# shaderko/velocity-asr

Measured on AMD Instinct MI355X. Metric: audio-sec/sec (RTFx) + frames/s, 5M model batch=32×10s @ 1/2/4/8 MI355X, higher is better.
Workload: dtype f32

## Files before the change

### velocity-asr_amd/csrc/gemm_rows.hip

```cpp
#include <type_traits>

#include "gemm_common.h"
#include "gemm_split.h"

namespace vasr {
namespace {

using namespace gemm;

typedef __attribute__((address_space(3))) void lds_void;

__device__ __forceinline__ void glds16(const void* src, void* dst_base) {
    const unsigned lds = (unsigned)(uintptr_t)(lds_void*)dst_base;
    unsigned keep;
    asm volatile("s_mov_b32 %0, m0\n\ts_mov_b32 m0, %1\n\ts_nop 0\n\tglobal_load_lds_dwordx4 %2, off\n\ts_mov_b32 m0, %0"
                 : "=&s"(keep) : "s"(lds), "v"(src) : "memory");
}

template <int N>
__device__ __forceinline__ void wait_vmcnt() {
    static_assert(N >= 0 && N < 64, "vmcnt range");
    __builtin_amdgcn_s_waitcnt((N & 15) | ((N >> 4) << 14) | (7 << 4) | (15 << 8));
}

#ifndef VASR_ROWS_ABLATE
#define VASR_ROWS_ABLATE 0
#endif
#ifndef VASR_ROWS_WAVES
#define VASR_ROWS_WAVES 8
#endif
#ifndef VASR_ROWS_DEPTH
#define VASR_ROWS_DEPTH 2
#endif
#ifndef VASR_ROWS_STORE_AUX
#define VASR_ROWS_STORE_AUX 2
#endif
constexpr int RW = VASR_ROWS_WAVES;
constexpr int DEPTH = VASR_ROWS_DEPTH;
constexpr int NSLOT = DEPTH + 1;
#ifndef VASR_ROWS_STORE_WAIT
#define VASR_ROWS_STORE_WAIT 1
#endif
#ifndef VASR_ROWS_MAX_GROUP
#define VASR_ROWS_MAX_GROUP 16
#endif
constexpr int MAX_GROUP = VASR_ROWS_MAX_GROUP;

__device__ __forceinline__ void wait_vmcnt_rt(int n) {
    switch (n) {
#define VASR_W(I) case I: wait_vmcnt<I>(); break;
#define VASR_W8(B) VASR_W(B) VASR_W(B + 1) VASR_W(B + 2) VASR_W(B + 3) VASR_W(B + 4) VASR_W(B + 5) VASR_W(B + 6) VASR_W(B + 7)
        VASR_W8(0) VASR_W8(8) VASR_W8(16) VASR_W8(24) VASR_W8(32) VASR_W8(40) VASR_W8(48) VASR_W8(56)
#undef VASR_W8
#undef VASR_W
        default: wait_vmcnt<0>();
    }
}

#ifdef VASR_ROWS_STAMPS
__device__ unsigned long long* g_rows_stamps;
#define VASR_STAMP(v) const unsigned long long v = __builtin_amdgcn_s_memtime()
#else
#define VASR_STAMP(v)
#endif

constexpr int NST = 16;
constexpr int OOB = 0x7FFFFFFC;

template <int EPI>
__device__ __forceinline__ void rows_epilogue(const GemmParams& p, __amdgpu_buffer_rsrc_t cbuf, int m0, int n0,
                                              const floatx16& acc, int r, int h, const float* __restrict__ bias_s,
                                              const float4* __restrict__ qp_s, int cfirst) {
    const int col = n0 + r;
    const bool col_ok = col < p.N;
    const int lc = col - cfirst;
    const float bv = p.bias ? bias_s[lc] : 0.0f;
    float4 qc = make_float4(0.f, 0.f, 0.f, 0.f);
    if (p.qp) qc = qp_s[lc];
    if constexpr (EPI == VASR_EPI_ARGMAX) {
        const int slot = n0 / 32;
#pragma unroll
        for (int i = 0; i < 16; ++i) {
            const int row = m0 + (i & 3) + 8 * (i >> 2) + 4 * h;
            float v = acc[i];
            if (p.bias) v = v + bv;
            if (p.qp) v = fake_quant(v, qc);
            const unsigned u = __float_as_uint(v);
            const unsigned ord = (u & 0x80000000u) ? ~u : (u | 0x80000000u);
            const unsigned long long k0 = col_ok ? ((unsigned long long)ord << 32) | (0xFFFFFFFFu - (unsigned)col) : 0ull;
            const unsigned long long key = gemm::max_u64_over_32_lanes(k0);
            const int off = (r == 31 && row < p.M) ? (row * (int)p.ldc + slot) * 8 : OOB;
            typedef unsigned u32x2 __attribute__((ext_vector_type(2)));
            const u32x2 kv = {(unsigned)key, (unsigned)(key >> 32)};
            if (!(VASR_ROWS_ABLATE & 2)) __builtin_amdgcn_raw_buffer_store_b64(kv, cbuf, off, 0, VASR_ROWS_STORE_AUX);
        }
        return;
    }
    auto body = [&](auto SPc) {
        constexpr int SP = decltype(SPc)::value;
        const bool sp = SP == 1 || (SP == 2 && col >= p.n_out);
#pragma unroll
        for (int i = 0; i < 16; ++i) {
            const int row = m0 + (i & 3) + 8 * (i >> 2) + 4 * h;
            const bool ok = col_ok && row < p.M;
            float v = acc[i];
            if (p.bias) v = v + bv;
            if (p.qp) v = fake_quant(v, qc);
            if constexpr (EPI == VASR_EPI_GELU) {
                v = gelu_fast(v);
            } else if constexpr (EPI == VASR_EPI_SOFTPLUS_FROM) {
                if constexpr (SP == 1) v = softplus20_fast(v);
                else if constexpr (SP == 2) v = sp ? softplus20_fast(v) : v;
            } else if constexpr (EPI == VASR_EPI_RESIDUAL) {
                v = v + p.aux[(int64_t)min(row, p.M - 1) * p.ld_aux + min(col, p.N - 1)];
            } else if constexpr (EPI == VASR_EPI_GELU_PE) {
                v = gelu_fast(v) + p.aux[(int64_t)min(row, p.M - 1) * p.ld_aux + min(col, p.N - 1)];
            }
            if (!(VASR_ROWS_ABLATE & 2))
                __builtin_amdgcn_raw_buffer_store_b32(__float_as_uint(v), cbuf, ok ? (row * (int)p.ldc + col) * 4 : OOB,
                                                      0, VASR_ROWS_STORE_AUX);
        }
    };
    if constexpr (EPI == VASR_EPI_SOFTPLUS_FROM) {
        if (n0 >= p.n_out) body(std::integral_constant<int, 1>());
        else if (n0 + 32 <= p.n_out) body(std::integral_constant<int, 0>());
        else body(std::integral_constant<int, 2>());
    } else {
        body(std::integral_constant<int, 0>());
    }
}

template <int KS, int EPI>
__global__ __launch_bounds__(64 * RW, 1) void gemm_rows_kernel(GemmParams p, int n_groups, int chunks_per_group) {
    constexpr int CHUNK = KS * 3 * 1024;
    constexpr int DW = 4;
    constexpr int NDMA = 3 * KS / DW;
    static_assert((3 * KS) % DW == 0 && RW % DW == 0, "whole DMA pieces per loader wave");
    __shared__ __attribute__((aligned(16))) char wb0[CHUNK];
    __shared__ __attribute__((aligned(16))) char wb1[CHUNK];
    __shared__ __attribute__((aligned(16))) char wb2[CHUNK];
    __shared__ __attribute__((aligned(16))) char wb3[NSLOT > 3 ? CHUNK : 16];
    __shared__ float bias_s[MAX_GROUP * 32];
    __shared__ float4 qp_s[MAX_GROUP * 32];

    const int nblk = (int)gridDim.x;
    const int id = blockIdx.x;
    const int q8 = nblk / 8, r8 = nblk % 8, xg = id % 8;
    const int w = (xg < r8 ? xg * (q8 + 1) : r8 * (q8 + 1) + (xg - r8) * q8) + id / 8;
    const int rb = w / n_groups, ng = w - rb * n_groups;
    const int NT = (p.N + 31) / 32;
    const int c0 = ng * chunks_per_group;
    const int nc = min(chunks_per_group, NT - c0);
    if (nc <= 0) return;

    const int tid = threadIdx.x;
    const int lane = tid & 63;
    const int wave = tid >> 6;
    const int r = lane & 31, h = lane >> 5;
    const int wave_u = __builtin_amdgcn_readfirstlane(wave);
    const int m0 = rb * 32 * RW + wave * 32;
    const int cfirst = c0 * 32;

    const float* __restrict__ arow = p.A + (int64_t)min(m0 + r, p.M - 1) * p.lda;
    float4 xa[KS][2];
#pragma unroll
    for (int ks = 0; ks < KS; ++ks)
#pragma unroll
        for (int u = 0; u < 2; ++u) {
            const int k = 16 * ks + 8 * h + 4 * u;
            const float4 v = *reinterpret_cast<const float4*>(arow + min(k, p.K - 4));
            xa[ks][u] = k < p.K ? v : make_float4(0.f, 0.f, 0.f, 0.f);
        }
    for (int i = tid; i < nc * 32; i += 64 * RW) {
        const int col = min(cfirst + i, p.N - 1);
        if (p.bias) bias_s[i] = p.bias[col];
        if (p.qp) qp_s[i] = p.qp[col];
    }
    bf16x8 a[KS][3];
#pragma unroll
    for (int ks = 0; ks < KS; ++ks) split8(xa[ks][0], xa[ks][1], a[ks][0], a[ks][1], a[ks][2]);

    const char* __restrict__ Wx = reinterpret_cast<const char*>(p.Wx);
    auto slot = [&](int i) -> char* { return i == 0 ? wb0 : i == 1 ? wb1 : i == 2 ? wb2 : wb3; };
    const bool loader = wave_u < DW;
    auto issue = [&](int j) {
        if (!loader) return;
        const char* src = Wx + (int64_t)(c0 + j) * CHUNK + lane * 16;
        char* dst = slot(j % NSLOT);
#pragma unroll
        for (int i = 0; i < NDMA; ++i) {
            const int piece = i * DW + wave_u;
            glds16(src + piece * 1024, dst + piece * 1024);
        }
    };
    for (int j = 0; j < DEPTH && j < nc; ++j) issue(j);

    const int c_bytes = (EPI == VASR_EPI_ARGMAX ? 8 : 4) * ((p.M - 1) * (int)p.ldc + (EPI == VASR_EPI_ARGMAX ? NT : p.N));
    const __amdgpu_buffer_rsrc_t cbuf = __builtin_amdgcn_make_buffer_rsrc(p.C, 0, c_bytes, 0x00020000);
    floatx16 acc[2];
#ifdef VASR_ROWS_STAMPS
    unsigned long long st_wait = 0, st_bar = 0, st_epi = 0, st_dma = 0, st_mfma = 0;
    VASR_STAMP(st_begin);
#endif
    auto step = [&](auto Sc, int j) {
        constexpr int S = decltype(Sc)::value;
        int n_vm = 0;
        if (!loader && !(VASR_ROWS_ABLATE & 2)) n_vm = VASR_ROWS_STORE_WAIT ? NST * max(0, j - max(j - DEPTH + 1, 1)) : 63;
        VASR_STAMP(t0);
        wait_vmcnt_rt(min(n_vm, 63));
        VASR_STAMP(t1);
        if (!(VASR_ROWS_ABLATE & 8)) __builtin_amdgcn_s_barrier();
        VASR_STAMP(t2);
        const char* wb = slot((VASR_ROWS_ABLATE & 4) ? min(j, DEPTH - 1) : j % NSLOT) + lane * 16;
        bf16x8 wf[2][3];
#pragma unroll
        for (int pl = 0; pl < 3; ++pl) wf[0][pl] = *reinterpret_cast<const bf16x8*>(wb + pl * 1024);
        if (j >= 1) rows_epilogue<EPI>(p, cbuf, m0, (c0 + j - 1) * 32, acc[S ^ 1], r, h, bias_s, qp_s, cfirst);
        VASR_STAMP(t3);
        if (j + DEPTH < nc && !(VASR_ROWS_ABLATE & 4)) issue(j + DEPTH);
        VASR_STAMP(t4);
        floatx16 c;
#pragma unroll
        for (int i = 0; i < 16; ++i) c[i] = 0.f;
#pragma unroll
        for (int ks = 0; ks < KS; ++ks) {
            const int cur = ks & 1;
            if (ks + 1 < KS) {
#pragma unroll
                for (int pl = 0; pl < 3; ++pl)
                    wf[cur ^ 1][pl] = *reinterpret_cast<const bf16x8*>(wb + ((ks + 1) * 3 + pl) * 1024);
            }
            __builtin_amdgcn_sched_barrier(0);
            if constexpr (VASR_ROWS_ABLATE & 1) {
                c[0] += (float)a[ks][0][0] * (float)wf[cur][0][0] + (float)a[ks][2][1] * (float)wf[cur][2][1];
                continue;
            }
            c = __builtin_amdgcn_mfma_f32_32x32x16_bf16(a[ks][2], wf[cur][0], c, 0, 0, 0);
            c = __builtin_amdgcn_mfma_f32_32x32x16_bf16(a[ks][0], wf[cur][2], c, 0, 0, 0);
            c = __builtin_amdgcn_mfma_f32_32x32x16_bf16(a[ks][1], wf[cur][1], c, 0, 0, 0);
            c = __builtin_amdgcn_mfma_f32_32x32x16_bf16(a[ks][1], wf[cur][0], c, 0, 0, 0);
            c = __builtin_amdgcn_mfma_f32_32x32x16_bf16(a[ks][0], wf[cur][1], c, 0, 0, 0);
            c = __builtin_amdgcn_mfma_f32_32x32x16_bf16(a[ks][0], wf[cur][0], c, 0, 0, 0);
            __builtin_amdgcn_sched_barrier(0);
        }
        acc[S] = c;
#ifdef VASR_ROWS_STAMPS
        VASR_STAMP(t5);
        st_wait += t1 - t0;
        st_bar += t2 - t1;
        st_epi += t3 - t2;
        st_dma += t4 - t3;
        st_mfma += t5 - t4;
#endif
    };
    for (int j = 0; j < nc; j += 2) {
        step(std::integral_constant<int, 0>(), j);
        if (j + 1 < nc) step(std::integral_constant<int, 1>(), j + 1);
    }
    const int jl = nc - 1;
    rows_epilogue<EPI>(p, cbuf, m0, (c0 + jl) * 32, (jl & 1) ? acc[1] : acc[0], r, h, bias_s, qp_s, cfirst);
#ifdef VASR_ROWS_STAMPS
    __builtin_amdgcn_s_waitcnt(0);
    VASR_STAMP(st_end);
    if (lane == 0 && g_rows_stamps) {
        unsigned long long* o = g_rows_stamps + ((int64_t)blockIdx.x * RW + wave) * 8;
        o[0] = st_wait; o[1] = st_bar; o[2] = st_epi; o[3] = st_dma; o[4] = st_mfma; o[5] = st_end - st_begin;
        o[6] = (unsigned long long)nc; o[7] = loader ? 1 : 0;
    }
#endif
}

template <int KS>
int launch_rows(const GemmParams& p, int epi, hipStream_t s) {
    const int NT = (p.N + 31) / 32;
    const int row_blocks = (p.M + 32 * RW - 1) / (32 * RW);
    int groups = 1, per = min(NT, MAX_GROUP), best = -1;
    for (int g = 1; g <= NT; ++g) {
        const int pg = (NT + g - 1) / g;
        if (pg > MAX_GROUP) continue;
        const int gg = (NT + pg - 1) / pg;
        const int cost = ((row_blocks * gg + kCUs - 1) / kCUs) * (pg + 1);
        if (best < 0 || cost < best) {
            best = cost;
            groups = gg;
            per = pg;
        }
    }
    const dim3 grid(row_blocks * groups), block(64 * RW);
#define VASR_R(E) hipLaunchKernelGGL((gemm_rows_kernel<KS, E>), grid, block, 0, s, p, groups, per)
    switch (epi) {
        case VASR_EPI_NONE: VASR_R(VASR_EPI_NONE); break;
        case VASR_EPI_GELU: VASR_R(VASR_EPI_GELU); break;
        case VASR_EPI_SOFTPLUS_FROM: VASR_R(VASR_EPI_SOFTPLUS_FROM); break;
        case VASR_EPI_RESIDUAL: VASR_R(VASR_EPI_RESIDUAL); break;
        case VASR_EPI_GELU_PE: VASR_R(VASR_EPI_GELU_PE); break;
        case VASR_EPI_ARGMAX: VASR_R(VASR_EPI_ARGMAX); break;
        default: set_error("vasr_linear_x3_f32: rows engine: epilogue %d not supported", epi); return VASR_EINVAL;
    }
#undef VASR_R
    return launch_status("vasr_linear_x3_f32");
}

}

bool try_rows_x3(const GemmParams& p, int batch, int epi, hipStream_t s, int* rc) {
    if (batch != 1 || p.Kp > 192 || p.M <= 0 || epi == VASR_EPI_PAIR_POWER || epi == VASR_EPI_PAIR_FUSION) return false;
    if (p.Kp != 128 && p.Kp != 192) return false;
    if ((int64_t)p.M * p.ldc * (epi == VASR_EPI_ARGMAX ? 8 : 4) >= ((int64_t)1 << 31) - 64) return false;
    const int engine = option(VASR_OPT_GEMM_ENGINE);
    if (engine == 1) return false;
    if (engine == 0 && (p.Kp != 192 || p.N < 512 || p.M < 4096 ||
                        !(epi == VASR_EPI_NONE || epi == VASR_EPI_GELU || epi == VASR_EPI_SOFTPLUS_FROM)))
        return false;
    *rc = p.Kp == 128 ? launch_rows<8>(p, epi, s) : launch_rows<12>(p, epi, s);
    return true;
}

}

#ifdef VASR_ROWS_STAMPS
VASR_API int vasr_diag_rows_stamps(void* buf) {
    return hipMemcpyToSymbol(HIP_SYMBOL(vasr::g_rows_stamps), &buf, sizeof(buf)) == hipSuccess ? VASR_OK : VASR_EINVAL;
}
#endif
```

Baseline: 159,500.

## Add warp-specialized rows GEMM kernel with separate compute, DMA and store waves

Adds a new rows GEMM kernel that splits each block into four MFMA compute waves and four memory waves. The memory waves issue global-to-LDS weight DMA into a three-slot ring and write the epilogue from a staged LDS tile, so stores and loads can overlap the matrix math. Weight chunks are interleaved across groups, blocks are remapped across XCDs, and wide 128-bit buffer stores are used when alignment allows. This is enabled by default, at the cost of more LDS per block, extra barriers and an extra LDS staging pass for the output.

After: 165,100 (median of 6 runs). +3.5%, better.

```diff
diff --git a/velocity-asr_amd/csrc/gemm_rows.hip b/velocity-asr_amd/csrc/gemm_rows.hip
--- a/velocity-asr_amd/csrc/gemm_rows.hip
+++ b/velocity-asr_amd/csrc/gemm_rows.hip
@@ -270,10 +270,306 @@
 #endif
 }
 
-template <int KS>
-int launch_rows(const GemmParams& p, int epi, hipStream_t s) {
+#ifndef VASR_ROWS_ROLES
+#define VASR_ROWS_ROLES 1
+#endif
+#ifndef VASR_ROWS_INTERLEAVE
+#define VASR_ROWS_INTERLEAVE 1
+#endif
+#ifndef VASR_ROWS_EPI_FIRST
+#define VASR_ROWS_EPI_FIRST 1
+#endif
+#ifndef VASR_ROWS_DMA_WAVES
+#define VASR_ROWS_DMA_WAVES 4
+#endif
+constexpr int CWV = 4;
+constexpr int MWV = 4;
+constexpr int DWV = VASR_ROWS_DMA_WAVES;
+constexpr int SWV = DWV == MWV ? MWV : MWV - DWV;
+static_assert(DWV == 4 || DWV == 2, "VASR_ROWS_DMA_WAVES: 4 or 2");
+constexpr int OOB16 = 0x7FFFFFF0;
+
+__device__ __forceinline__ void role_barrier() {
+    asm volatile("" ::: "memory");
+    __builtin_amdgcn_s_barrier();
+    asm volatile("" ::: "memory");
+}
+
+template <int EPI, int SP>
+__device__ __forceinline__ float rows_value(const GemmParams& p, float v, float bv, const float4& qc, int row, int col) {
+    if (p.bias) v = v + bv;
+    if (p.qp) v = fake_quant(v, qc);
+    if constexpr (EPI == VASR_EPI_GELU) {
+        v = gelu_fast(v);
+    } else if constexpr (EPI == VASR_EPI_SOFTPLUS_FROM) {
+        if constexpr (SP == 1) v = softplus20_fast(v);
+        else if constexpr (SP == 2) v = col >= p.n_out ? softplus20_fast(v) : v;
+    } else if constexpr (EPI == VASR_EPI_RESIDUAL) {
+        v = v + p.aux[(int64_t)min(row, p.M - 1) * p.ld_aux + min(col, p.N - 1)];
+    } else if constexpr (EPI == VASR_EPI_GELU_PE) {
+        v = gelu_fast(v) + p.aux[(int64_t)min(row, p.M - 1) * p.ld_aux + min(col, p.N - 1)];
+    }
+    return v;
+}
+
+template <int EPI>
+__device__ __forceinline__ void roles_epilogue(const GemmParams& p, __amdgpu_buffer_rsrc_t cbuf, int m0, int n0,
+                                               const float* __restrict__ tile, int lane, bool wide,
+                                               const float* __restrict__ bias_s, const float4* __restrict__ qp_s,
+                                               int cfirst) {
+    const int rl = lane >> 3, c4 = 4 * (lane & 7);
+    const int col0 = n0 + c4;
+    const int lc = col0 - cfirst;
+    float bv[4] = {0.f, 0.f, 0.f, 0.f};
+    if (p.bias) {
+        const float4 b = *reinterpret_cast<const float4*>(bias_s + lc);
+        bv[0] = b.x; bv[1] = b.y; bv[2] = b.z; bv[3] = b.w;
+    }
+    float4 qc[4];
+#pragma unroll
+    for (int e = 0; e < 4; ++e) qc[e] = p.qp ? qp_s[lc + e] : make_float4(0.f, 0.f, 0.f, 0.f);
+    if constexpr (EPI == VASR_EPI_ARGMAX) {
+        const int slot = n0 / 32;
+#pragma unroll
+        for (int s = 0; s < 4; ++s) {
+            const int row = m0 + 8 * s + rl;
+            const float4 x = *reinterpret_cast<const float4*>(tile + (8 * s + rl) * 32 + c4);
+            const float xv[4] = {x.x, x.y, x.z, x.w};
+            unsigned long long key = 0ull;
+#pragma unroll
+            for (int e = 0; e < 4; ++e) {
+                float v = xv[e];
+                if (p.bias) v = v + bv[e];
+                if (p.qp) v = fake_quant(v, qc[e]);
+                const unsigned u = __float_as_uint(v);
+                const unsigned ord = (u & 0x80000000u) ? ~u : (u | 0x80000000u);
+                const unsigned long long k =
+                    col0 + e < p.N ? ((unsigned long long)ord << 32) | (0xFFFFFFFFu - (unsigned)(col0 + e)) : 0ull;
+                key = k > key ? k : key;
+            }
+            unsigned long long o = gemm::dpp_u64<0xB1, 0xF>(key);
+            key = o > key ? o : key;
+            o = gemm::dpp_u64<0x4E, 0xF>(key);
+            key = o > key ? o : key;
+            o = gemm::dpp_u64<0x141, 0xF>(key);
+            key = o > key ? o : key;
+            const int off = (c4 == 0 && row < p.M) ? (row * (int)p.ldc + slot) * 8 : OOB16;
+            typedef unsigned u32x2 __attribute__((ext_vector_type(2)));
+            const u32x2 kv = {(unsigned)key, (unsigned)(key >> 32)};
+            __builtin_amdgcn_raw_buffer_store_b64(kv, cbuf, off, 0, VASR_ROWS_STORE_AUX);
+        }
+        return;
+    }
+    auto body = [&](auto SPc, auto Wc) {
+        constexpr int SP = decltype(SPc)::value;
+        constexpr bool WIDE = decltype(Wc)::value;
+#pragma unroll
+        for (int s = 0; s < 4; ++s) {
+            const int row = m0 + 8 * s + rl;
+            const float4 x = *reinterpret_cast<const float4*>(tile + (8 * s + rl) * 32 + c4);
+            float v[4] = {x.x, x.y, x.z, x.w};
+#pragma unroll
+            for (int e = 0; e < 4; ++e) v[e] = rows_value<EPI, SP>(p, v[e], bv[e], qc[e], row, col0 + e);
+            if constexpr (WIDE) {
+                typedef unsigned u32x4 __attribute__((ext_vector_type(4)));
+                const u32x4 d = {__float_as_uint(v[0]), __float_as_uint(v[1]), __float_as_uint(v[2]), __float_as_uint(v[3])};
+                const int off = (row < p.M && col0 < p.N) ? (row * (int)p.ldc + col0) * 4 : OOB16;
+                if (!(VASR_ROWS_ABLATE & 2) || s == 3) __builtin_amdgcn_raw_buffer_store_b128(d, cbuf, off, 0, VASR_ROWS_STORE_AUX);
+            } else {
+#pragma unroll
+                for (int e = 0; e < 4; ++e)
+                    __builtin_amdgcn_raw_buffer_store_b32(__float_as_uint(v[e]), cbuf,
+                                                          (row < p.M && col0 + e < p.N) ? (row * (int)p.ldc + col0 + e) * 4 : OOB,
+                                                          0, VASR_ROWS_STORE_AUX);
+            }
+        }
+    };
+    auto width = [&](auto SPc) {
+        if (wide) body(SPc, std::true_type());
+        else body(SPc, std::false_type());
+    };
+    if constexpr (EPI == VASR_EPI_SOFTPLUS_FROM) {
+        if (n0 >= p.n_out) width(std::integral_constant<int, 1>());
+        else if (n0 + 32 <= p.n_out) width(std::integral_constant<int, 0>());
+        else width(std::integral_constant<int, 2>());
+    } else {
+        width(std::integral_constant<int, 0>());
+    }
+}
+
+template <int KS, int EPI>
+__global__ __launch_bounds__(64 * (CWV + MWV), 1) void gemm_rows_roles_kernel(GemmParams p, int n_groups,
+                                                                              int chunks_per_group, int wide) {
+    constexpr int CHUNK = KS * 3 * 1024;
+    constexpr int NDMA = 3 * KS / DWV;
+    static_assert((3 * KS) % DWV == 0, "whole DMA pieces per DMA wave");
+    static_assert(DEPTH == 2, "the roles kernel's ring is three slots, two chunks ahead");
+    __shared__ __attribute__((aligned(16))) char wb0[CHUNK];
+    __shared__ __attribute__((aligned(16))) char wb1[CHUNK];
+    __shared__ __attribute__((aligned(16))) char wb2[CHUNK];
+    __shared__ __attribute__((aligned(16))) float stage[CWV][2][1024];
+    __shared__ __attribute__((aligned(16))) float bias_s[MAX_GROUP * 32];
+    __shared__ float4 qp_s[MAX_GROUP * 32];
+
+    const int nblk = (int)gridDim.x;
+    const int id = blockIdx.x;
+    const int q8 = nblk / 8, r8 = nblk % 8, xg = id % 8;
+    const int w = (xg < r8 ? xg * (q8 + 1) : r8 * (q8 + 1) + (xg - r8) * q8) + id / 8;
+    const int rb = w / n_groups, ng = w - rb * n_groups;
     const int NT = (p.N + 31) / 32;
-    const int row_blocks = (p.M + 32 * RW - 1) / (32 * RW);
+    constexpr bool IL = VASR_ROWS_INTERLEAVE != 0;
+    const int c0 = IL ? ng : ng * chunks_per_group, cstep = IL ? n_groups : 1;
+    const int nc = IL ? (NT - ng + n_groups - 1) / n_groups : min(chunks_per_group, NT - c0);
+    if (nc <= 0) return;
+
+    const int tid = threadIdx.x;
+    const int lane = tid & 63;
+    const int wave_u = __builtin_amdgcn_readfirstlane(tid >> 6);
+    auto slot = [&](int i) -> char* { return i == 0 ? wb0 : i == 1 ? wb1 : wb2; };
+#ifdef VASR_ROWS_STAMPS
+    unsigned long long st_wait = 0, st_bar = 0, st_epi = 0, st_dma = 0, st_mfma = 0;
+    VASR_STAMP(st_begin);
+#endif
+
+    if (wave_u < CWV) {
+        const int r = lane & 31, h = lane >> 5;
+        const int m0 = rb * 32 * CWV + wave_u * 32;
+        const float* __restrict__ arow = p.A + (int64_t)min(m0 + r, p.M - 1) * p.lda;
+        float4 xa[KS][2];
+#pragma unroll
+        for (int ks = 0; ks < KS; ++ks)
+#pragma unroll
+            for (int u = 0; u < 2; ++u) {
+                const int k = 16 * ks + 8 * h + 4 * u;
+                const float4 v = *reinterpret_cast<const float4*>(arow + min(k, p.K - 4));
+                xa[ks][u] = k < p.K ? v : make_float4(0.f, 0.f, 0.f, 0.f);
+            }
+        bf16x8 a[KS][3];
+#pragma unroll
+        for (int ks = 0; ks < KS; ++ks) split8(xa[ks][0], xa[ks][1], a[ks][0], a[ks][1], a[ks][2]);
+        for (int j = 0; j < nc; ++j) {
+            VASR_STAMP(t0);
+            role_barrier();
+            VASR_STAMP(t1);
+            const char* wb = slot(j % NSLOT) + lane * 16;
+            bf16x8 wf[2][3];
+#pragma unroll
+            for (int pl = 0; pl < 3; ++pl) wf[0][pl] = *reinterpret_cast<const bf16x8*>(wb + pl * 1024);
+            floatx16 c;
+#pragma unroll
+            for (int i = 0; i < 16; ++i) c[i] = 0.f;
+#pragma unroll
+            for (int ks = 0; ks < KS; ++ks) {
+                const int cur = ks & 1;
+                if (ks + 1 < KS) {
+#pragma unroll
+                    for (int pl = 0; pl < 3; ++pl)
+                        wf[cur ^ 1][pl] = *reinterpret_cast<const bf16x8*>(wb + ((ks + 1) * 3 + pl) * 1024);
+                }
+                __builtin_amdgcn_sched_barrier(0);
+                c = __builtin_amdgcn_mfma_f32_32x32x16_bf16(a[ks][2], wf[cur][0], c, 0, 0, 0);
+                c = __builtin_amdgcn_mfma_f32_32x32x16_bf16(a[ks][0], wf[cur][2], c, 0, 0, 0);
+                c = __builtin_amdgcn_mfma_f32_32x32x16_bf16(a[ks][1], wf[cur][1], c, 0, 0, 0);
+                c = __builtin_amdgcn_mfma_f32_32x32x16_bf16(a[ks][1], wf[cur][0], c, 0, 0, 0);
+                c = __builtin_amdgcn_mfma_f32_32x32x16_bf16(a[ks][0], wf[cur][1], c, 0, 0, 0);
+                c = __builtin_amdgcn_mfma_f32_32x32x16_bf16(a[ks][0], wf[cur][0], c, 0, 0, 0);
+                __builtin_amdgcn_sched_barrier(0);
+            }
+            VASR_STAMP(t2);
+            float* tile = &stage[wave_u][j & 1][0];
+#pragma unroll
+            for (int i = 0; i < 16; ++i) tile[((i & 3) + 8 * (i >> 2) + 4 * h) * 32 + r] = c[i];
+            __builtin_amdgcn_s_waitcnt(0xC07F);
+#ifdef VASR_ROWS_STAMPS
+            VASR_STAMP(t3);
+            st_bar += t1 - t0;
+            st_mfma += t2 - t1;
+            st_epi += t3 - t2;
+#endif
+        }
+        VASR_STAMP(t4);
+        role_barrier();
+#ifdef VASR_ROWS_STAMPS
+        VASR_STAMP(t5);
+        st_bar += t5 - t4;
+#endif
+    } else {
+        const int mw = wave_u - CWV;
+        const bool dma = mw < DWV;
+        const bool stores = mw >= MWV - SWV;
+        const int sw = mw - (MWV - SWV);
+        for (int i = tid - 64 * CWV; i < nc * 32; i += 64 * MWV) {
+            const int col = min((c0 + (i >> 5) * cstep) * 32 + (i & 31), p.N - 1);
+            if (p.bias) bias_s[i] = p.bias[col];
+            if (p.qp) qp_s[i] = p.qp[col];
+        }
+        const char* __restrict__ Wx = reinterpret_cast<const char*>(p.Wx);
+        auto issue = [&](int j) {
+            const char* src = Wx + (int64_t)(c0 + j * cstep) * CHUNK + lane * 16;
+            char* dst = slot(j % NSLOT);
+#pragma unroll
+            for (int i = 0; i < NDMA; ++i) {
+                const int piece = i * DWV + mw;
+                glds16(src + piece * 1024, dst + piece * 1024);
+            }
+        };
+        __builtin_amdgcn_s_waitcnt(0xC07F);
+        if (dma)
+            for (int j = 0; j < DEPTH && j < nc; ++j) issue(j);
+        const int c_bytes = (EPI == VASR_EPI_ARGMAX ? 8 : 4) * ((p.M - 1) * (int)p.ldc + (EPI == VASR_EPI_ARGMAX ? NT : p.N));
+        const __amdgpu_buffer_rsrc_t cbuf = __builtin_amdgcn_make_buffer_rsrc(p.C, 0, c_bytes, 0x00020000);
+        auto epilogue = [&](int j) {
+            if (!stores) return;
+            const int n0 = (c0 + j * cstep) * 32;
+            for (int cw = sw; cw < CWV; cw += SWV)
+                roles_epilogue<EPI>(p, cbuf, rb * 32 * CWV + cw * 32, n0, &stage[cw][j & 1][0], lane, wide != 0,
+                                    bias_s, qp_s, n0 - j * 32);
+        };
+        for (int j = 0; j < nc; ++j) {
+            VASR_STAMP(t0);
+            if (dma) {
+                if (j + 1 < nc) wait_vmcnt<NDMA*(DEPTH - 1)>();
+                else wait_vmcnt<0>();
+            }
+            VASR_STAMP(t1);
+            role_barrier();
+            VASR_STAMP(t2);
+            if (VASR_ROWS_EPI_FIRST && j >= 1) epilogue(j - 1);
+            VASR_STAMP(t2e);
+            if (dma && j + DEPTH < nc && !(VASR_ROWS_ABLATE & 4)) issue(j + DEPTH);
+            VASR_STAMP(t3);
+            if (!VASR_ROWS_EPI_FIRST && j >= 1) epilogue(j - 1);
+#ifdef VASR_ROWS_STAMPS
+            VASR_STAMP(t4);
+            st_wait += t1 - t0;
+            st_bar += t2 - t1;
+            st_dma += t3 - t2e;
+            st_epi += (t2e - t2) + (t4 - t3);
+#endif
+        }
+        VASR_STAMP(t5);
+        role_barrier();
+        VASR_STAMP(t6);
+        epilogue(nc - 1);
+#ifdef VASR_ROWS_STAMPS
+        VASR_STAMP(t7);
+        st_bar += t6 - t5;
+        st_epi += t7 - t6;
+#endif
+    }
+#ifdef VASR_ROWS_STAMPS
+    __builtin_amdgcn_s_waitcnt(0);
+    VASR_STAMP(st_end);
+    if (lane == 0 && g_rows_stamps) {
+        unsigned long long* o = g_rows_stamps + ((int64_t)blockIdx.x * (CWV + MWV) + wave_u) * 8;
+        o[0] = st_wait; o[1] = st_bar; o[2] = st_epi; o[3] = st_dma; o[4] = st_mfma; o[5] = st_end - st_begin;
+        o[6] = (unsigned long long)nc;
+        o[7] = wave_u < CWV ? 2 : DWV == MWV ? 3 : wave_u - CWV < DWV ? 4 : 5;
+    }
+#endif
+}
+
+inline void pick_groups(int row_blocks, int NT, int* groups_out, int* per_out) {
     int groups = 1, per = min(NT, MAX_GROUP), best = -1;
     for (int g = 1; g <= NT; ++g) {
         const int pg = (NT + g - 1) / g;
@@ -286,6 +582,38 @@
             per = pg;
         }
     }
+    *groups_out = groups;
+    *per_out = per;
+}
+
+template <int KS>
+int launch_roles(const GemmParams& p, int epi, hipStream_t s) {
+    const int NT = (p.N + 31) / 32;
+    const int row_blocks = (p.M + 32 * CWV - 1) / (32 * CWV);
+    int groups, per;
+    pick_groups(row_blocks, NT, &groups, &per);
+    const int wide = epi != VASR_EPI_ARGMAX && p.N % 4 == 0 && p.ldc % 4 == 0 && (reinterpret_cast<uintptr_t>(p.C) & 15) == 0;
+    const dim3 grid(row_blocks * groups), block(64 * (CWV + MWV));
+#define VASR_R(E) hipLaunchKernelGGL((gemm_rows_roles_kernel<KS, E>), grid, block, 0, s, p, groups, per, wide)
+    switch (epi) {
+        case VASR_EPI_NONE: VASR_R(VASR_EPI_NONE); break;
+        case VASR_EPI_GELU: VASR_R(VASR_EPI_GELU); break;
+        case VASR_EPI_SOFTPLUS_FROM: VASR_R(VASR_EPI_SOFTPLUS_FROM); break;
+        case VASR_EPI_RESIDUAL: VASR_R(VASR_EPI_RESIDUAL); break;
+        case VASR_EPI_GELU_PE: VASR_R(VASR_EPI_GELU_PE); break;
+        case VASR_EPI_ARGMAX: VASR_R(VASR_EPI_ARGMAX); break;
+        default: set_error("vasr_linear_x3_f32: rows engine: epilogue %d not supported", epi); return VASR_EINVAL;
+    }
+#undef VASR_R
+    return launch_status("vasr_linear_x3_f32");
+}
+
+template <int KS>
+int launch_rows(const GemmParams& p, int epi, hipStream_t s) {
+    const int NT = (p.N + 31) / 32;
+    const int row_blocks = (p.M + 32 * RW - 1) / (32 * RW);
+    int groups, per;
+    pick_groups(row_blocks, NT, &groups, &per);
     const dim3 grid(row_blocks * groups), block(64 * RW);
 #define VASR_R(E) hipLaunchKernelGGL((gemm_rows_kernel<KS, E>), grid, block, 0, s, p, groups, per)
     switch (epi) {
@@ -312,7 +640,9 @@
     if (engine == 0 && (p.Kp != 192 || p.N < 512 || p.M < 4096 ||
                         !(epi == VASR_EPI_NONE || epi == VASR_EPI_GELU || epi == VASR_EPI_SOFTPLUS_FROM)))
         return false;
-    *rc = p.Kp == 128 ? launch_rows<8>(p, epi, s) : launch_rows<12>(p, epi, s);
+    const bool roles = VASR_ROWS_ROLES != 0;
+    if (roles) *rc = p.Kp == 128 ? launch_roles<8>(p, epi, s) : launch_roles<12>(p, epi, s);
+    else *rc = p.Kp == 128 ? launch_rows<8>(p, epi, s) : launch_rows<12>(p, epi, s);
     return true;
 }
 
```
